# abdelhakim96/Dynamic-Obstacle-Avoidance-MPC

Measured on AMD Instinct MI355X. Metric: MPC solves/sec (N=20, 3 obstacles), higher is better.
Workload: dtype f64; 1 GPU; C2: 1024 identical scenarios per GPU, N=20, Tf=2s, 3 moving obstacles; global_batch=1024, per_gpu_batch=1024, N=20, n_obst=3, parallelism=single GPU

## Files before the change

### dynamic-obstacle-avoidance-mpc_amd/csrc/rti_split_kernel.hpp

```cpp
#pragma once
#include "rti_kernel.hpp"
#include <type_traits>

namespace mpc {

template <int LPS, int NOBST, bool W2 = false, bool BLK2 = false>
struct SplitLds {
    using LT = typename std::conditional<W2, RowLdsC, RowLds>::type;
    static constexpr int NBL = 6 / LPS;
    static constexpr int NSL = (NOBST + LPS - 1) / LPS;
    static __host__ __device__ constexpr int results(int N) { return W2 ? 0 : (N + 1) * RowLds::HS; }
    static __host__ __device__ constexpr int total(int N, bool lookahead)
    {
        if (BLK2) return Blk2Lds::total(N) + (lookahead ? (N + 1) * NOBST * 2 : 0);
        return LT::total(N, 1) + results(N) + ((lookahead && !W2) ? (N + 1) * NOBST * 2 : 0);
    }
};

template <int K>
__device__ __forceinline__ double nth_of_six(double a0, double a1, double a2, double a3, double a4, double a5)
{
    if constexpr (K == 0) return a0; else if constexpr (K == 1) return a1; else if constexpr (K == 2) return a2;
    else if constexpr (K == 3) return a3; else if constexpr (K == 4) return a4; else return a5;
}

#ifdef MPC_FORCE_WAVES2
#define MPC_SPLIT_BOUNDS(W2) __launch_bounds__(64, 2)
#else
#define MPC_SPLIT_BOUNDS(W2) __launch_bounds__(64, (W2) ? 2 : 1)
#endif
template <int NOBST, int LPS, bool W2 = false, bool MASKED = false, bool BLK2 = false, bool REF = false, bool IPAR = false, bool OSEL = false, bool IBND = false, bool NSQP = false>
__global__ MPC_SPLIT_BOUNDS(W2) void rti_split_kernel(const KParams p)
{
    static_assert(!NSQP || (IBND && !W2 && !BLK2), "the SQP loop is built on the per-instance bounds' code (dense blocks, one wavefront per SIMD)");
    static_assert(!IBND || OSEL, "the per-instance bounds are built on the obstacle masks' code");
    static_assert(!OSEL || (IPAR && MASKED), "the obstacle masks are built on the per-instance parameters' code with a run-time row count");
    static_assert(!REF || !BLK2, "the per-stage reference is not built for the block-2 recursions");
    static_assert(!IPAR || REF, "the per-instance parameters are built on the per-stage reference's code");
    static_assert(LPS == 2 || LPS == 3, "two or three lanes per horizon stage");
    static_assert(!BLK2 || !W2, "the block-2 recursions exist on the dense layout only");
    using SL = SplitLds<LPS, NOBST, W2, BLK2>;
    using LT = typename SL::LT;
    constexpr int NBL = SL::NBL, NSL = SL::NSL;
    constexpr int kKK = 45;
    const int lane = threadIdx.x;
    const int inst = p.order ? p.order[blockIdx.x] : (int)blockIdx.x;
    const int N = p.N;
    const int nact = MASKED ? p.n_obst : NOBST;
    const int i = lane / LPS;
    const int h = lane - i * LPS;
    const bool own = (h == 0);
    uint32_t omask = 0u;
    if constexpr (OSEL) omask = omask_word(p.omask, __builtin_amdgcn_readfirstlane(inst), nact);
    const int osub = OSEL ? 31 - __builtin_clz(omask | 1u) : 0;
#define OBST_ON(j) (OSEL ? (((omask >> (j)) & 1u) != 0u) : ((j) < nact))
#define OBST_IN(j) (OSEL ? ((((omask >> (j)) & 1u) != 0u) ? (j) : osub) : ((j) < nact ? (j) : nact - 1))
    const bool act = (i <= N);
    const bool has_u = (i < N);
    const bool xb = (i >= 1) && (i < N || (i == N && p.bx_terminal));
    const double dt = p.dt, h2 = p.h2;
    int is_part1 = (h == 1), is_part2 = (h == 2);
    asm volatile("" : "+v"(is_part1), "+v"(is_part2));
    auto part_of = [&](auto sc, double a0, double a1, double a2, double a3, double a4, double a5) {
        constexpr int s = decltype(sc)::value;
        double r = nth_of_six<s>(a0, a1, a2, a3, a4, a5);
        r = is_part1 ? nth_of_six<NBL + s>(a0, a1, a2, a3, a4, a5) : r;
        if (LPS == 3) r = is_part2 ? nth_of_six<(2 * NBL + s) % 6>(a0, a1, a2, a3, a4, a5) : r;
        return r;
    };
    auto zpart_of = [&](auto sc, double v0, double v1, double v2, double v3, double v5, double v6) {
        return part_of(sc, v0, v1, v2, v3, v5, v6);
    };
    using slot0 = std::integral_constant<int, 0>; using slot1 = std::integral_constant<int, 1>; using slot2 = std::integral_constant<int, 2>;
    auto slots_of = [&](const double (&v)[7], double (&out)[NBL]) {
        out[0] = zpart_of(slot0{}, v[0], v[1], v[2], v[3], v[5], v[6]);
        out[1] = zpart_of(slot1{}, v[0], v[1], v[2], v[3], v[5], v[6]);
        if constexpr (NBL > 2) out[2] = zpart_of(slot2{}, v[0], v[1], v[2], v[3], v[5], v[6]);
    };

#ifdef MPC_PHASE_TIMING
    long long tacc_[16] = {0, 0, 0, 0, 0, 0, 0, 0, 0, 0, 0, 0, 0, 0, 0, 0};
#endif
    MPC_T0();
    double x0v[5], gl[2];
#pragma unroll
    for (int c = 0; c < 5; c++) x0v[c] = p.x0[(size_t)inst * 5 + c];
    gl[0] = p.goal[(size_t)inst * 2]; gl[1] = p.goal[(size_t)inst * 2 + 1];
    if constexpr (W2) {
#pragma unroll
        for (int c = 0; c < 5; c++) x0v[c] = wave_uniform(x0v[c]);
        gl[0] = wave_uniform(gl[0]); gl[1] = wave_uniform(gl[1]);
    }
    double *Xg = p.X + (size_t)inst * (N + 1) * 5, *Ug = p.U + (size_t)inst * N * 2;
    const int ep_word = ((p.fused & kFuseMetrics) && p.ep_flags) ? p.ep_flags[inst] : 0;
    double xi[5] = {0, 0, 0, 0, 0}, ui[2] = {0, 0}, xnext[5] = {0, 0, 0, 0, 0};
    if (act) {
#pragma unroll
        for (int c = 0; c < 5; c++) xi[c] = Xg[i * 5 + c];
    }
    if (has_u) {
        ui[0] = Ug[i * 2]; ui[1] = Ug[i * 2 + 1];
#pragma unroll
        for (int c = 0; c < 5; c++) xnext[c] = Xg[(i + 1) * 5 + c];
    }
    extern __shared__ double lds_raw[];
    const LT RL = [&]() {
        if constexpr (W2) return RowLdsC(lds_raw + RowLdsC::CT + RowLdsC::pad_front(N), N, lds_raw);
        else return RowLds(lds_raw + RowLds::pad_front(N), N, lds_raw + RowLds::total(N, 1));
    }();
    const Blk2Lds BL(lds_raw, N);
    const RowLds RV(lds_raw, N / 2, BL.R);
    const int Mb = N >> 1;
    const int mblk = i >> 1;
    const bool odd = (i & 1) != 0;
    double *lds_P = BLK2 ? lds_raw + Blk2Lds::total(N) : (W2 ? RL.H : lds_raw + LT::total(N, 1) + SL::results(N));
    auto of_part = [&](double v, int q) { return q == 0 ? v : (q == 1 ? from_right(v) : from_right(from_right(v))); };
    constexpr bool FX = !W2 && !BLK2 && !(LPS == 2 && NOBST > 5);
    const bool obst_step = p.obst && (p.fused & (kFusePlant | kFuseObstacles | kFuseMetrics)) && lane < nact;
    double og[4] = {0, 0, 0, 0}, onz[2] = {0, 0};
    if constexpr (FX) {
        if (obst_step) {
            const double *o = p.obst + ((size_t)inst * nact + lane) * 4;
#pragma unroll
            for (int c = 0; c < 4; c++) og[c] = o[c];
            if ((p.fused & kFuseObstacles) && p.noise) { onz[0] = p.noise[((size_t)inst * nact + lane) * 2]; onz[1] = p.noise[((size_t)inst * nact + lane) * 2 + 1]; }
        }
    }
    double pxy[NSL][2];
    if (p.obst) {
        if (lane < 2 * nact) {
            const int j = lane >> 1, c = lane & 1;
            const double *o = p.obst + ((size_t)inst * nact + j) * 4;
            double q = o[c], v = (c == 0 && !p.world.bug_compat_predict) ? o[2] : o[3];
            const double lo = c ? p.world.ymin : p.world.xmin, hi = c ? p.world.ymax : p.world.xmax;
            lds_P[lane] = q;
            int k = 1;
            if constexpr (FX) {
                for (; k + 3 <= N; k += 4) {
                    double q4[4];
                    if (coord_advance4_clear(lo, hi, dt, q, v, q4)) q = q4[3];
                    else {
#pragma unroll
                        for (int j = 0; j < 4; j++) { coord_advance(lo, hi, dt, q, v); q4[j] = q; }
                    }
#pragma unroll
                    for (int j = 0; j < 4; j++) lds_P[(k + j) * NOBST * 2 + lane] = q4[j];
                }
            }
            for (; k <= N; k++) {
                coord_advance(lo, hi, dt, q, v);
                lds_P[k * NOBST * 2 + lane] = q;
            }
        }
        wave_sync();
    }
    MPC_TICK(10);
    if (p.obst) {
#pragma unroll
        for (int s = 0; s < NSL; s++) {
            const int j = s * LPS + h, jj = OBST_IN(j);
            const double *src = lds_P + ((act ? i : 0) * NOBST + jj) * 2;
            pxy[s][0] = src[0]; pxy[s][1] = src[1];
        }
    } else {
#pragma unroll
        for (int s = 0; s < NSL; s++) {
            const int j = s * LPS + h, jj = OBST_IN(j);
            const double *src = p.P + (((size_t)inst * (N + 1) + (act ? i : 0)) * nact + jj) * 2;
            pxy[s][0] = src[0]; pxy[s][1] = src[1];
        }
    }
    if constexpr (OSEL) {
        if (omask == 0u) {
#pragma unroll
            for (int s = 0; s < NSL; s++) { pxy[s][0] = 0.0; pxy[s][1] = 0.0; }
        }
    }
    if constexpr (FX) {
        if (p.obst) wave_sync();
        if (obst_step) {
            if (p.fused & kFuseObstacles) {
                if (p.noise) obstacle_noise(p.randomness, p.vmax, onz[0], onz[1], og[2], og[3]);
                obstacle_advance(p.world, dt, og[0], og[2], og[1], og[3]);
            }
            double *w = lds_P + 4 * lane;
#pragma unroll
            for (int c = 0; c < 4; c++) w[c] = og[c];
        }
    }
    const bool ep_done = (ep_word & 1) != 0;
    [[maybe_unused]] int sqp_k = 0, sqp_it = 0;
sqp_again: ;
    double fin = gl[0] + gl[1] + ui[0] + ui[1];
#pragma unroll
    for (int c = 0; c < 5; c++) fin += x0v[c] + xi[c] + xnext[c];
#pragma unroll
    for (int s = 0; s < NSL; s++) fin += pxy[s][0] + pxy[s][1];

    MPC_TICK(11);
    double zpen = 0.0;
    {
        const double ex = x0v[0] - gl[0], ey = x0v[1] - gl[1];
        const double scale = p.slack_a * (ex * ex + ey * ey + x0v[3] * x0v[3] + x0v[4] * x0v[4] + p.slack_b);
        const double alpha_i = p.alpha ? p.alpha[(size_t)inst * (N + 1) + (act ? i : N)] : scale * (double)(N - i) / (double)N;
        zpen = alpha_i * (has_u ? p.ss : 1.0);
    }
    const bool vs = act && (i >= 1) && (p.soft_h ? (zpen > 0.0) : true);
    const bool soft = p.soft_h != 0;

    double lin0 = 0.0;
    double d0[5] = {0, 0, 0, 0, 0};
    StageLin S;
    S.a02 = S.a03 = S.a04 = S.a12 = S.a13 = S.a14 = S.b00 = S.b01 = S.b10 = S.b11 = 0.0; S.dt = dt; S.h2 = h2;
    double bb[5] = {0, 0, 0, 0, 0};
    if (has_u) {
        double xn[5], ae[6], be[4];
        dyn_step<true>(xi, ui, dt, xn, ae, be);
        S.a02 = ae[0]; S.a03 = ae[1]; S.a04 = ae[2]; S.a12 = ae[3]; S.a13 = ae[4]; S.a14 = ae[5];
        S.b00 = be[0]; S.b01 = be[1]; S.b10 = be[2]; S.b11 = be[3];
#pragma unroll
        for (int c = 0; c < 5; c++) { bb[c] = xn[c] - xnext[c]; lin0 = fmax(lin0, fabs(bb[c])); }
    }
    if (i == 0) {
#pragma unroll
        for (int c = 0; c < 5; c++) { d0[c] = x0v[c] - xi[c]; lin0 = fmax(lin0, fabs(d0[c])); }
    }
    StageLin Sa = S;
    double bba[5] = {0, 0, 0, 0, 0}, bh0[5] = {0, 0, 0, 0, 0};
    if constexpr (BLK2) {
        if (own && has_u) {
            double *w = BL.S + 16 * i;
            w[0] = bb[2]; w[1] = bb[3]; w[2] = S.a02; w[3] = S.a03; w[4] = S.a04; w[5] = bb[0]; w[6] = S.b00; w[7] = S.b01;
            w[8] = bb[4]; w[9] = 0.0; w[10] = S.a12; w[11] = S.a13; w[12] = S.a14; w[13] = bb[1]; w[14] = S.b10; w[15] = S.b11;
        }
        wave_sync();
        if (act && odd) {
            const double *w = BL.S + 16 * (i - 1);
            Sa.a02 = w[2]; Sa.a03 = w[3]; Sa.a04 = w[4]; Sa.b00 = w[6]; Sa.b01 = w[7];
            Sa.a12 = w[10]; Sa.a13 = w[11]; Sa.a14 = w[12]; Sa.b10 = w[14]; Sa.b11 = w[15];
            bba[0] = w[5]; bba[1] = w[13]; bba[2] = w[0]; bba[3] = w[1]; bba[4] = w[8];
        }
        if (own && odd && has_u) {
            const double Wh[5][10] = {
                {1.0, 0.0, Sa.a02 + S.a02, Sa.a03 + S.a03, fma(S.a02, dt, Sa.a04) + S.a04, 0.0,
                 fma(S.a03, dt, Sa.b00), fma(S.a04, dt, fma(S.a02, h2, Sa.b01)), S.b00, S.b01},
                {0.0, 1.0, Sa.a12 + S.a12, Sa.a13 + S.a13, fma(S.a12, dt, Sa.a14) + S.a14, 0.0,
                 fma(S.a13, dt, Sa.b10), fma(S.a14, dt, fma(S.a12, h2, Sa.b11)), S.b10, S.b11},
                {0.0, 0.0, 1.0, 0.0, 2.0 * dt, 0.0, 0.0, fma(dt, dt, h2), 0.0, h2},
                {0.0, 0.0, 0.0, 1.0, 0.0, 0.0, dt, 0.0, dt, 0.0},
                {0.0, 0.0, 0.0, 0.0, 1.0, 0.0, 0.0, dt, 0.0, dt}};
            double *w = BL.W + Blk2Lds::WS * mblk;
#pragma unroll
            for (int k = 0; k < 5; k++)
#pragma unroll
                for (int c = 0; c < 10; c++) w[k * 10 + c] = Wh[k][c];
            bh0[0] = fma(S.a04, bba[4], fma(S.a03, bba[3], fma(S.a02, bba[2], bba[0]))) + bb[0];
            bh0[1] = fma(S.a14, bba[4], fma(S.a13, bba[3], fma(S.a12, bba[2], bba[1]))) + bb[1];
            bh0[2] = fma(dt, bba[4], bba[2]) + bb[2]; bh0[3] = bba[3] + bb[3]; bh0[4] = bba[4] + bb[4];
        }
        if (own && act && (odd || i == N)) {
            double *hc = BL.H + Blk2Lds::HS * mblk;
#pragma unroll
            for (int e = 0; e < 100; e++) hc[e] = 0.0;
        }
    } else
    if constexpr (W2) {
        if (own && act) { double *hc = RL.H + LT::HS * i; hc[49] = 0.0; hc[50] = 0.0; }
        if (lane < 8) {
            const double c2[8] = {0.0, 0.0, 1.0, 0.0, dt, 0.0, 0.0, h2}, c3[8] = {0.0, 0.0, 0.0, 1.0, 0.0, 0.0, dt, 0.0}, c4[8] = {0.0, 0.0, 0.0, 0.0, 1.0, 0.0, 0.0, dt};
            double v2 = 0.0, v3 = 0.0, v4 = 0.0;
// ... 31 lines not shown
    double cl0[NBL], ch0[NBL], hq[NBL], hd[NBL], gc0[NBL];
    double ll[NBL], tl[NBL], lh[NBL], th[NBL], rtl[NBL], rth[NBL], zs[NBL];
    double yr[REF ? 6 : 1];
    if constexpr (IPAR) load_ref_or_goal<IPAR>(p.yref, p.ref_off, p.ref_T, inst, act ? i : N, has_u, gl, yr);
    else if constexpr (REF) load_ref(p, inst, act ? i : N, has_u, yr);
    IpConst *const ipw = IPAR ? ip_const(p.ip_w, (size_t)__builtin_amdgcn_readfirstlane(inst) * kIpW) : nullptr;
#define ROW_R2(s) (IPAR ? p.ip_r2[(size_t)inst * nact + (OSEL ? OBST_IN((s) * LPS + h) : ((s) * LPS + h < nact ? (s) * LPS + h : nact - 1))] : p.r2)
    IpConst *const ipb = IBND ? ip_const(p.ip_b, (size_t)__builtin_amdgcn_readfirstlane(inst) * kIpB) : nullptr;
    {
        auto slot_init = [&](auto sc) {
            constexpr int s = decltype(sc)::value;
            const double val = part_of(sc, ui[0], ui[1], xi[0], xi[1], xi[3], xi[4]);
            double lo, hi;
            if constexpr (IBND) {
                lo = part_of(sc, ipb[kIpBuLo + 0], ipb[kIpBuLo + 1], ipb[kIpBxLo + 0], ipb[kIpBxLo + 1], ipb[kIpBxLo + 2], ipb[kIpBxLo + 3]);
                hi = part_of(sc, ipb[kIpBuHi + 0], ipb[kIpBuHi + 1], ipb[kIpBxHi + 0], ipb[kIpBxHi + 1], ipb[kIpBxHi + 2], ipb[kIpBxHi + 3]);
            } else {
                lo = part_of(sc, p.bu_lo[0], p.bu_lo[1], p.bx_lo[0], p.bx_lo[1], p.bx_lo[2], p.bx_lo[3]);
                hi = part_of(sc, p.bu_hi[0], p.bu_hi[1], p.bx_hi[0], p.bx_hi[1], p.bx_hi[2], p.bx_hi[3]);
            }
            const bool is_u = part_of(sc, 1.0, 1.0, 0.0, 0.0, 0.0, 0.0) != 0.0;
            bp[s] = act && (is_u ? has_u : xb);
            if constexpr (IPAR)
                hd[s] = part_of(sc, has_u ? ipw[kIpHs + 0] : 0.0, has_u ? ipw[kIpHs + 1] : 0.0, has_u ? ipw[kIpHs + 2] : ipw[kIpHt + 0],
                                has_u ? ipw[kIpHs + 3] : ipw[kIpHt + 1], has_u ? ipw[kIpHs + 5] : ipw[kIpHt + 3], has_u ? ipw[kIpHs + 6] : ipw[kIpHt + 4]);
            else
                hd[s] = part_of(sc, has_u ? p.Hd_stage[0] : 0.0, has_u ? p.Hd_stage[1] : 0.0, has_u ? p.Hd_stage[2] : p.Hd_term[0],
                                has_u ? p.Hd_stage[3] : p.Hd_term[1], has_u ? p.Hd_stage[5] : p.Hd_term[3], has_u ? p.Hd_stage[6] : p.Hd_term[4]);
            hq[s] = (is_u && !has_u) ? 1.0 : hd[s];
            double wg;
            if constexpr (IPAR)
                wg = part_of(sc, has_u ? ipw[kIpWg + 4] : 0.0, has_u ? ipw[kIpWg + 5] : 0.0, has_u ? ipw[kIpWg + 0] : ipw[kIpWe + 0], has_u ? ipw[kIpWg + 1] : ipw[kIpWe + 1],
                             has_u ? ipw[kIpWg + 2] : ipw[kIpWe + 2], has_u ? ipw[kIpWg + 3] : ipw[kIpWe + 3]);
            else
                wg = part_of(sc, has_u ? p.Wg[4] : 0.0, has_u ? p.Wg[5] : 0.0, has_u ? p.Wg[0] : p.Weg[0], has_u ? p.Wg[1] : p.Weg[1],
                             has_u ? p.Wg[2] : p.Weg[2], has_u ? p.Wg[3] : p.Weg[3]);
            if constexpr (REF) gc0[s] = wg * (val - part_of(sc, yr[4], yr[5], yr[0], yr[1], yr[2], yr[3]));
            else gc0[s] = wg * (val - part_of(sc, 0.0, 0.0, gl[0], gl[1], 0.0, 0.0));
            cl0[s] = val - lo; ch0[s] = hi - val;
            tl[s] = fmax(cl0[s], p.thr0); th[s] = fmax(ch0[s], p.thr0);
            rtl[s] = rcp_nr(tl[s]); rth[s] = rcp_nr(th[s]);
            ll[s] = p.mu0 * rtl[s]; lh[s] = p.mu0 * rth[s];
            zs[s] = 0.0;
            if (bp[s]) lin0 = fmax(lin0, fmax(tl[s] - cl0[s], th[s] - ch0[s]));
        };
        slot_init(std::integral_constant<int, 0>{});
        slot_init(std::integral_constant<int, 1>{});
        if constexpr (NBL > 2) slot_init(std::integral_constant<int, 2>{});
    }
    double hd_psi_;
    if constexpr (IPAR) hd_psi_ = has_u ? ipw[kIpHs + 4] : ipw[kIpHt + 2];
    else hd_psi_ = has_u ? p.Hd_stage[4] : p.Hd_term[2];
    const double hd_psi = hd_psi_;
    bool sp[NSL];
    double hh[NSL], ax[NSL], ay[NSL], sv[NSL], l1[NSL], t1[NSL], l2[NSL], t2[NSL], rt1[NSL], rt2[NSL];
#pragma unroll
    for (int s = 0; s < NSL; s++) {
        if constexpr (OSEL) sp[s] = vs && OBST_ON(s * LPS + h);
        else sp[s] = vs && (s * LPS + h < nact);
        const double ex = xi[0] - pxy[s][0], ey = xi[1] - pxy[s][1];
        hh[s] = ex * ex + ey * ey - ROW_R2(s); ax[s] = 2 * ex; ay[s] = 2 * ey;
        if (soft) {
            sv[s] = (hh[s] < 0 ? -hh[s] : 0.0) + p.thr0;
            t1[s] = fmax(hh[s] + sv[s], p.thr0);
            t2[s] = fmax(sv[s], p.thr0);
        } else {
            sv[s] = 0.0; t1[s] = fmax(hh[s], p.thr0); t2[s] = 1.0;
            if (sp[s]) lin0 = fmax(lin0, t1[s] - hh[s]);
        }
        rt1[s] = rcp_nr(t1[s]); rt2[s] = rcp_nr(t2[s]);
        l1[s] = p.mu0 * rt1[s]; l2[s] = soft ? p.mu0 * rt2[s] : 0.0;
    }
    int n_items_lane = 0;
#pragma unroll
    for (int s = 0; s < NBL; s++) n_items_lane += bp[s] ? 2 : 0;
#pragma unroll
    for (int s = 0; s < NSL; s++) n_items_lane += sp[s] ? (soft ? 2 : 1) : 0;
    const double n_items = seg_sum<64>((double)n_items_lane, lane);
    const double inv_items = wave_uniform(n_items > 0 ? 1.0 / n_items : 0.0);
    if (!(fabs(fin) <= 1e300)) lin0 = INFINITY;
    lin0 = wave_uniform(seg_max<64>(lin0, lane));

    double z[7] = {0, 0, 0, 0, 0, 0, 0};
    double rhoPi = 1.0;
    int it = 0;
    IpmState ipm;
    ipm.running = !ep_done;
    int &status = ipm.status, &it_done = ipm.it_done;
    bool &running = ipm.running;
    float stepl = 0.0f;
    if (!(lin0 <= 1e300)) { status = 4; running = false; }

    auto stationarity = [&]() {
        double gsh[NBL], gk[6] = {0, 0, 0, 0, 0, 0}, sx = 0.0, sy = 0.0, rsm = 0.0;
#pragma unroll
        for (int s = 0; s < NBL; s++) { gsh[s] = gc0[s] + hd[s] * zs[s] + (bp[s] ? lh[s] - ll[s] : 0.0); gk[s] = gsh[s]; }
#pragma unroll
        for (int s = 0; s < NSL; s++) if (sp[s]) {
            sx -= l1[s] * ax[s]; sy -= l1[s] * ay[s];
            if (soft) rsm = fmax(rsm, fabs(zpen * sv[s] + zpen - l1[s] - l2[s]));
        }
        double shx = sx, shy = sy;
#pragma unroll
        for (int q = 1; q < LPS; q++) {
#pragma unroll
            for (int s = 0; s < NBL; s++) gsh[s] = from_right(gsh[s]);
// ... 39 lines not shown
        double rdl[NBL], rdh[NBL];
        struct SoftT { double w1, w2, rD, be1, be2, rs, rd1, rd2; } so[NSL];
        double hdiag_[NBL], g_[NBL], ssum[5];
        {
#pragma unroll
            for (int s = 0; s < NBL; s++) {
                rdl[s] = (cl0[s] + zs[s]) - tl[s];
                rdh[s] = (ch0[s] - zs[s]) - th[s];
                double hdiag = hq[s], g = gc0[s] + hd[s] * zs[s];
                if (bp[s]) {
                    const double wl = ll[s] * rtl[s], wh = lh[s] * rth[s];
                    const double bl = (ll[s] * tl[s] + ll[s] * rdl[s]) * rtl[s], bh = (lh[s] * th[s] + lh[s] * rdh[s]) * rth[s];
                    hdiag += wl + wh;
                    g += lh[s] - ll[s];
                    g += bl - bh;
                }
                hdiag_[s] = hdiag; g_[s] = g;
            }
            double sxx = 0.0, syy = 0.0, sxy = 0.0, glx = 0.0, gly = 0.0, cbx = 0.0, cby = 0.0;
#pragma unroll
            for (int s = 0; s < NSL; s++) {
                SoftT &o = so[s];
                const double y = ax[s] * z[2] + ay[s] * z[3];
                o.w1 = l1[s] * rt1[s];
                if (soft) {
                    o.rd1 = (hh[s] + y + sv[s]) - t1[s]; o.rd2 = sv[s] - t2[s];
                    o.be1 = (l1[s] * t1[s] + l1[s] * o.rd1) * rt1[s];
                    o.w2 = l2[s] * rt2[s];
                    o.be2 = (l2[s] * t2[s] + l2[s] * o.rd2) * rt2[s];
                    o.rs = zpen * sv[s] + zpen - l1[s] - l2[s];
                    o.rD = rcp_nr(zpen + o.w1 + o.w2);
                } else {
                    o.rd1 = (hh[s] + y) - t1[s]; o.rd2 = 0.0;
                    o.be1 = (l1[s] * t1[s] + l1[s] * o.rd1) * rt1[s];
                    o.w2 = 0.0; o.be2 = 0.0; o.rs = 0.0; o.rD = 0.0;
                }
                if (sp[s]) {
                    double weff, geff;
                    if (soft) {
                        weff = o.w1 * (zpen + o.w2) * o.rD;
                        geff = (o.be1 * (zpen + o.w2) - o.w1 * (o.rs + o.be2)) * o.rD;
                    } else { weff = o.w1; geff = o.be1; }
                    sxx += weff * ax[s] * ax[s]; syy += weff * ay[s] * ay[s]; sxy += weff * ax[s] * ay[s];
                    glx -= l1[s] * ax[s]; gly -= l1[s] * ay[s];
                    cbx += geff * ax[s]; cby += geff * ay[s];
                }
            }
            ssum[0] = sxx; ssum[1] = syy; ssum[2] = sxy; ssum[3] = glx + cbx; ssum[4] = gly + cby;
        }
        MPC_TICK(1);
        double bbr[5], x_init[5];
#pragma unroll
        for (int c = 0; c < 5; c++) { bbr[c] = rhoPi * bb[c]; x_init[c] = rhoPi * d0[c]; }
        {
            double Hk[6], gk[6], Ssum[5], sh_h[NBL], sh_g[NBL], sh_s[5];
#pragma unroll
            for (int s = 0; s < NBL; s++) { Hk[s] = hdiag_[s]; gk[s] = g_[s]; sh_h[s] = hdiag_[s]; sh_g[s] = g_[s]; }
#pragma unroll
            for (int e = 0; e < 5; e++) { Ssum[e] = ssum[e]; sh_s[e] = ssum[e]; }
#pragma unroll
            for (int q = 1; q < LPS; q++) {
#pragma unroll
                for (int s = 0; s < NBL; s++) { sh_h[s] = from_right(sh_h[s]); sh_g[s] = from_right(sh_g[s]); }
#pragma unroll
                for (int e = 0; e < 5; e++) sh_s[e] = from_right(sh_s[e]);
#pragma unroll
                for (int s = 0; s < NBL; s++) { Hk[q * NBL + s] = sh_h[s]; gk[q * NBL + s] = sh_g[s]; }
#pragma unroll
                for (int e = 0; e < 5; e++) Ssum[e] += sh_s[e];
            }
            const double Sxx = Ssum[0], Syy = Ssum[1], Sxy = Ssum[2], Sgx = Ssum[3], Sgy = Ssum[4];
            if constexpr (BLK2) {
                const double q[5] = {Hk[2] + Sxx, Hk[3] + Syy, hd_psi, Hk[4], Hk[5]};
                const double g[5] = {gk[2] + Sgx, gk[3] + Sgy, hd_psi * z[4], gk[4], gk[5]};
                const double r0 = Hk[0], r1 = Hk[1], lu0 = gk[0], lu1 = gk[1];
                if (own && act && !odd && i < N) {
                    double *x = BL.R + Blk2Lds::RS * mblk;
#pragma unroll
                    for (int c = 0; c < 5; c++) { x[c] = q[c]; x[5 + c] = g[c]; }
                    x[10] = Sxy; x[11] = r0; x[12] = r1; x[13] = lu0; x[14] = lu1;
                }
                if (own && i == N) {
                    double *hc = BL.H + Blk2Lds::HS * mblk;
#pragma unroll
                    for (int c = 0; c < 5; c++) { hc[11 * c] = q[c]; hc[10 * c + 5] = g[c]; hc[50 + c] = g[c]; }
                    hc[1] = Sxy; hc[10] = Sxy;
                }
                wave_sync();
                if (own && odd && act) {
                    const double *x = BL.R + Blk2Lds::RS * mblk;
                    double qa[5], ga[5];
#pragma unroll
                    for (int c = 0; c < 5; c++) { qa[c] = x[c]; ga[c] = x[5 + c]; }
                    const double qaxy = x[10], ra0 = x[11], ra1 = x[12], lua0 = x[13], lua1 = x[14];
                    const double C0[7] = {1.0, 0.0, Sa.a02, Sa.a03, Sa.a04, Sa.b00, Sa.b01}, C1[7] = {0.0, 1.0, Sa.a12, Sa.a13, Sa.a14, Sa.b10, Sa.b11};
                    double s0[7], s1[7];
                    s0[0] = q[0]; s0[1] = Sxy; s1[0] = Sxy; s1[1] = q[1];
#pragma unroll
                    for (int c = 2; c < 7; c++) { s0[c] = fma(q[0], C0[c], Sxy * C1[c]); s1[c] = fma(Sxy, C0[c], q[1] * C1[c]); }
                    double Y[7][7];
#pragma unroll
                    for (int c = 0; c < 7; c++) { Y[0][c] = s0[c]; Y[1][c] = s1[c]; }
#pragma unroll
                    for (int r = 2; r < 7; r++)
#pragma unroll
                        for (int c = r; c < 7; c++) Y[r][c] = fma(C0[r], s0[c], C1[r] * s1[c]);
// ... 113 lines not shown
        if constexpr (BLK2) {
            rowpar_factor2(lane, Mb, BL, lane < 16);
            wave_sync();
            if (has_u) {
                const double *ko = BL.R + Blk2Lds::RS * mblk;
#pragma unroll
                for (int u = 0; u < 4; u++) {
#pragma unroll
                    for (int c = 0; c < 5; c++) Kh[u][c] = ko[8 * u + c];
                    kh[u] = ko[8 * u + 5];
                }
                if (own && odd) {
#pragma unroll
                    for (int e = 0; e < 10; e++) fac[e] = ko[Blk2Lds::FAC + e];
                }
            }
            if (own && odd && has_u) {
                const double B0[4] = {fma(S.a03, dt, Sa.b00), fma(S.a04, dt, fma(S.a02, h2, Sa.b01)), S.b00, S.b01};
                const double B1[4] = {fma(S.a13, dt, Sa.b10), fma(S.a14, dt, fma(S.a12, h2, Sa.b11)), S.b10, S.b11};
                const double A0[5] = {1.0, 0.0, Sa.a02 + S.a02, Sa.a03 + S.a03, fma(S.a02, dt, Sa.a04) + S.a04};
                const double A1[5] = {0.0, 1.0, Sa.a12 + S.a12, Sa.a13 + S.a13, fma(S.a12, dt, Sa.a14) + S.a14};
                const double h2d = fma(dt, dt, h2);
                double *acl = BL.R + Blk2Lds::RS * mblk + RowVec::ACL;
#pragma unroll
                for (int c = 0; c < 6; c++) {
                    const double k0 = c < 5 ? Kh[0][c] : kh[0], k1 = c < 5 ? Kh[1][c] : kh[1], k2 = c < 5 ? Kh[2][c] : kh[2], k3 = c < 5 ? Kh[3][c] : kh[3];
                    const double a0 = c < 5 ? A0[c] : rhoPi * bh0[0], a1 = c < 5 ? A1[c] : rhoPi * bh0[1];
                    const double a2 = c < 5 ? (c == 2 ? 1.0 : (c == 4 ? 2.0 * dt : 0.0)) : rhoPi * bh0[2];
                    const double a3 = c < 5 ? (c == 3 ? 1.0 : 0.0) : rhoPi * bh0[3], a4 = c < 5 ? (c == 4 ? 1.0 : 0.0) : rhoPi * bh0[4];
                    acl[0 * RowVec::RS + c] = fma(B0[3], k3, fma(B0[2], k2, fma(B0[1], k1, fma(B0[0], k0, a0))));
                    acl[1 * RowVec::RS + c] = fma(B1[3], k3, fma(B1[2], k2, fma(B1[1], k1, fma(B1[0], k0, a1))));
                    acl[2 * RowVec::RS + c] = fma(h2, k3, fma(h2d, k1, a2));
                    acl[3 * RowVec::RS + c] = fma(dt, k2, fma(dt, k0, a3));
                    acl[4 * RowVec::RS + c] = fma(dt, k3, fma(dt, k1, a4));
                }
            }
            MPC_TICK(2);
            if (lane == 0) {
#pragma unroll
                for (int c = 0; c < 5; c++) BL.R[RowVec::X + c] = x_init[c];
            }
            wave_sync();
            MPC_TICK(3);
            rowpar_vector_fast<true>(lane, Mb, RV, lane < 16);
            MPC_TICK(15);
            wave_sync();
            pair_step(bbra, za);
            MPC_TICK(3);
        } else {
#ifdef MPC_MFMA4
        if constexpr (!W2) mfma4_factor(lane, N, RL); else
#endif
        {
            constexpr bool kSixRows = W2 || (NOBST == 10 && LPS == 2 && !MASKED && REF && IPAR && !OSEL);
            rowpar_factor<LT, (LT::COMPACT ? kSweepTermsCopied : kSweepTermsOutOfPlace), kSixRows>(lane, N, RL, lane < 16, dt);
        }
        wave_sync();
        if (has_u) {
            const double *ko = RL.R + LT::HS * i;
#pragma unroll
            for (int c = 0; c < 5; c++) { F.K0[c] = ko[c]; F.K1[c] = ko[8 + c]; }
            F.k0 = ko[5]; F.k1 = ko[13]; F.i00 = ko[6]; F.l = ko[7]; F.i11 = ko[14];
        }
        if (own && has_u) {
            double *acl = RL.R + LT::HS * i + RowVec::ACL;
            const double Ar[2][5] = {{1.0, 0.0, S.a02, S.a03, S.a04}, {0.0, 1.0, S.a12, S.a13, S.a14}};
            const double Br[2][2] = {{S.b00, S.b01}, {S.b10, S.b11}};
#pragma unroll
            for (int c = 0; c < 5; c++) {
                acl[0 * RowVec::RS + c] = Ar[0][c] + Br[0][0] * F.K0[c] + Br[0][1] * F.K1[c];
                acl[1 * RowVec::RS + c] = Ar[1][c] + Br[1][0] * F.K0[c] + Br[1][1] * F.K1[c];
                acl[2 * RowVec::RS + c] = (c == 2 ? 1.0 : (c == 4 ? dt : 0.0)) + h2 * F.K1[c];
                acl[3 * RowVec::RS + c] = (c == 3 ? 1.0 : 0.0) + dt * F.K0[c];
                acl[4 * RowVec::RS + c] = (c == 4 ? 1.0 : 0.0) + dt * F.K1[c];
            }
            double *cc = acl + 5;
            cc[0 * RowVec::RS] = bbr[0] + S.b00 * F.k0 + S.b01 * F.k1; cc[1 * RowVec::RS] = bbr[1] + S.b10 * F.k0 + S.b11 * F.k1;
            cc[2 * RowVec::RS] = bbr[2] + h2 * F.k1; cc[3 * RowVec::RS] = bbr[3] + dt * F.k0; cc[4 * RowVec::RS] = bbr[4] + dt * F.k1;
        }
        MPC_TICK(2);
        if (lane == 0) {
#pragma unroll
            for (int c = 0; c < 5; c++) RL.R[RowVec::X + c] = x_init[c];
        }
        wave_sync();
        MPC_TICK(3);
        rowpar_vector_fast<true>(lane, N, RL, lane < 16);
        MPC_TICK(15);
        wave_sync();
        if (act) {
            const double *xx = RL.R + LT::HS * i + RowVec::X;
            double u0 = F.k0, u1 = F.k1;
#pragma unroll
            for (int c = 0; c < 5; c++) { za[2 + c] = xx[c]; u0 += F.K0[c] * xx[c]; u1 += F.K1[c] * xx[c]; }
            za[0] = u0; za[1] = u1;
        }
        MPC_TICK(3);

        }

        double ppl[NBL], pph[NBL], pp1[NSL], pp2[NSL];
        double smu;
        {
            double rmax = 0.0, rmaxd = 0.0;
            double dtl_[NBL], dth_[NBL], dll_[NBL], dlh_[NBL], zas[NBL];
            slots_of(za, zas);
#pragma unroll
            for (int s = 0; s < NBL; s++) {
                const double dzk = zas[s];
                dtl_[s] = dzk + rdl[s]; dth_[s] = -dzk + rdh[s];
                dll_[s] = -(ll[s] * tl[s] + ll[s] * dtl_[s]) * rtl[s]; dlh_[s] = -(lh[s] * th[s] + lh[s] * dth_[s]) * rth[s];
                ppl[s] = dll_[s] * dtl_[s]; pph[s] = dlh_[s] * dth_[s];
                if (bp[s]) {
                    rmax = fmax(rmax, fmax(-dtl_[s] * rtl[s], -dth_[s] * rth[s]));
                    rmaxd = fmax(rmaxd, fmax(fma(dtl_[s], rtl[s], 1.0), fma(dth_[s], rth[s], 1.0)));
                }
// ... 256 lines not shown
        const double *xg = p.x0 + (size_t)inst * 5, *gg = p.goal + (size_t)inst * 2;
        asm volatile("" : "+v"(xg), "+v"(gg));
#pragma unroll
        for (int c = 0; c < 5; c++) x0v[c] = xg[c];
        gl[0] = gg[0]; gl[1] = gg[1];
    }
    if constexpr (NSQP) {
        status = ipm_finite_step<64>(status, z, lane);
        tail_full_step(status, z, xi, ui);
        sqp_k += 1; sqp_it += it_done;
        const double nrm = wave_uniform(seg_max<64>(sqp_step_norm(act, has_u, z), lane));
        if (!ep_done && status != 4 && sqp_k < p.sqp_max && !(nrm <= p.sqp_tol)) {
#pragma unroll
            for (int c = 0; c < 5; c++) {
                xi[c] = act ? xi[c] : 0.0;
                double r = from_right(xi[c]);
#pragma unroll
                for (int q = 1; q < LPS; q++) r = from_right(r);
                xnext[c] = has_u ? r : 0.0;
            }
            ui[0] = has_u ? ui[0] : 0.0; ui[1] = has_u ? ui[1] : 0.0;
            goto sqp_again;
        }
        it_done = sqp_it;
    }
    if constexpr (FX) {
        const bool store = !ep_done;
        const bool lane0s = (lane == 0) && store;
        double ox = 0.0, oy = 0.0, ovx = 0.0, ovy = 0.0;
        if (obst_step) {
            const double *w = lds_P + 4 * lane;
            ox = w[0]; oy = w[1]; ovx = w[2]; ovy = w[3];
        }
        int acc_it = 0, acc_st = 0, ep_fl = 0, ep_inc = 0;
        double ep_mm = 0.0;
        if (lane0s) {
            if (p.iters_acc) acc_it = p.iters_acc[inst];
            if (p.status_acc) acc_st = p.status_acc[inst];
            if (p.fused & kFuseMetrics) { ep_fl = p.ep_flags[inst]; ep_mm = p.ep_min_margin[inst]; }
        }
        if constexpr (!NSQP) {
        status = ipm_finite_step<64>(status, z, lane);
        tail_full_step(status, z, xi, ui);
        }
        const double u_apply[2] = {lane_value(ui[0], 0), lane_value(ui[1], 0)};
        tail_reset_on_fail(p.fused, status, x0v, gl[1], i, N, xi, ui);
        const bool fused_step = (p.fused & (kFusePlant | kFuseObstacles | kFuseMetrics)) != 0;
        double xnew[5] = {x0v[0], x0v[1], x0v[2], x0v[3], x0v[4]};
        if (fused_step) {
            double xp[5] = {x0v[0], x0v[1], x0v[2], x0v[3], x0v[4]};
            if ((p.fused & kFuseAliasBug) && (p.fused & kFuseResetOnFail) && status == 4) { xp[3] = 0.0; xp[4] = 0.0; }
#pragma unroll
            for (int c = 0; c < 5; c++) xnew[c] = xp[c];
            if (p.fused & kFusePlant) dyn_step<false>(xp, u_apply, dt, xnew, nullptr, nullptr);
            double margin = INFINITY;
            if (obst_step) {
                const double ddx = xnew[0] - ox, ddy = xnew[1] - oy;
                margin = sqrt(ddx * ddx + ddy * ddy) - (IPAR ? p.ip_rhit[(size_t)inst * nact + lane] : p.r_hit);
                if constexpr (OSEL) {
                    if (!OBST_ON(lane) && !(p.fused & kFuseMarginAll)) margin = INFINITY;
                }
            }
            if (p.fused & kFuseMetrics) {
                margin = -seg_max<64>(-margin, lane);
                if (lane0s) {
                    if (xnew[0] < p.world.xmin || xnew[0] > p.world.xmax || xnew[1] < p.world.ymin || xnew[1] > p.world.ymax) ep_fl |= 2;
                    ep_mm = fmin(ep_mm, margin);
                    if (ep_mm <= 0.0) ep_fl |= 4;
                    const double gx_ = xnew[0] - gl[0], gy_ = xnew[1] - gl[1];
                    if (sqrt(gx_ * gx_ + gy_ * gy_) <= p.tol_goal) ep_fl |= 1;
                    else ep_inc = 1;
                }
            }
        }
        double J = 0.0;
        if (p.cost) {
            if (act) {
                if (IPAR && own) {
                    double r[6];
                    load_ref_or_goal<IPAR>(p.yref, p.ref_off, p.ref_T, inst, i, has_u, gl, r);
                    const double wg[6] = {ipw[kIpWg], ipw[kIpWg + 1], ipw[kIpWg + 2], ipw[kIpWg + 3], ipw[kIpWg + 4], ipw[kIpWg + 5]};
                    const double we[4] = {ipw[kIpWe], ipw[kIpWe + 1], ipw[kIpWe + 2], ipw[kIpWe + 3]};
                    J = ls_cost_ref(wg, we, xi, ui, r, has_u);
                } else if (REF && own) {
                    const double *row = ref_row(p.yref, p.ref_off, p.ref_T, inst, i);
                    const double r[6] = {row[0], row[1], row[2], row[3], has_u ? row[4] : 0.0, has_u ? row[5] : 0.0};
                    J = ls_cost_ref(p.Wg, p.Weg, xi, ui, r, has_u);
                } else if (own) {
                    const double ex = xi[0] - gl[0], ey = xi[1] - gl[1];
                    if (has_u) J = 0.5 * (p.Wg[0] * ex * ex + p.Wg[1] * ey * ey + p.Wg[2] * xi[3] * xi[3] + p.Wg[3] * xi[4] * xi[4]
                                          + p.Wg[4] * ui[0] * ui[0] + p.Wg[5] * ui[1] * ui[1]);
                    else J = 0.5 * (p.Weg[0] * ex * ex + p.Weg[1] * ey * ey + p.Weg[2] * xi[3] * xi[3] + p.Weg[3] * xi[4] * xi[4]);
                }
#pragma unroll
                for (int s = 0; s < NSL; s++) if (OBST_ON(s * LPS + h)) {
                    const double dx = xi[0] - pxy[s][0], dy = xi[1] - pxy[s][1];
                    const double hv = dx * dx + dy * dy - ROW_R2(s);
                    const double v = hv < 0 ? -hv : 0.0;
                    J += zpen * (v + 0.5 * v * v);
                }
            }
            J = seg_sum<64>(J, lane);
        }
        if (store && own && (status != 4 || (p.fused & (kFuseResetOnFail | kFuseShift)))) tail_store_iterate(p.fused, i, N, act, has_u, xi, ui, Xg, Ug);
        if (fused_step) {
            if ((p.fused & kFusePlant) && lane0s && p.x0_rw) {
#pragma unroll
// ... 126 lines not shown
```

Baseline: 7.667 million solves/s.

## Spread dynamics quadrature, Hessian staging and closed-loop rows across lanes of each stage

Each lane of a horizon stage now computes only its share of the Gauss-Legendre quadrature sincos nodes and exchanges them with neighbours through cross-lane moves. This replaces every lane evaluating all four nodes redundantly in the linearisation and the plant step. Hessian and gradient staging into LDS and the closed-loop A+BK rows are also split so each lane writes its own entries, where one owner lane used to build everything. This trims redundant transcendental and serial work per stage, at the cost of extra cross-lane shuffles, selects and more intricate index bookkeeping that could be wrong for some template configurations.

```diff
diff --git a/dynamic-obstacle-avoidance-mpc_amd/csrc/rti_split_kernel.hpp b/dynamic-obstacle-avoidance-mpc_amd/csrc/rti_split_kernel.hpp
--- a/dynamic-obstacle-avoidance-mpc_amd/csrc/rti_split_kernel.hpp
+++ b/dynamic-obstacle-avoidance-mpc_amd/csrc/rti_split_kernel.hpp
@@ -22,6 +22,91 @@
 {
     if constexpr (K == 0) return a0; else if constexpr (K == 1) return a1; else if constexpr (K == 2) return a2;
     else if constexpr (K == 3) return a3; else if constexpr (K == 4) return a4; else return a5;
+}
+
+__device__ __forceinline__ void dyn_step_quad(const double x[5], const double u[2], double dt, int lane, double xn[5])
+{
+    const double psi = x[2], v = x[3], om = x[4], a = u[0], al = u[1];
+    double vj[4], pj[4], w[4];
+#pragma unroll
+    for (int j = 0; j < 4; j++) {
+        const double tau = kGLC[j] * dt;
+        w[j] = kGLB[j] * dt;
+        vj[j] = v + a * tau;
+        pj[j] = psi + om * tau + 0.5 * al * tau * tau;
+    }
+    const int k = lane & 3;
+    double arg = pj[0];
+    arg = (k == 1) ? pj[1] : arg; arg = (k == 2) ? pj[2] : arg; arg = (k == 3) ? pj[3] : arg;
+    double sk, ck;
+    sincos(arg, &sk, &ck);
+    const double sn[4] = {dpp_f64<0x00>(sk), dpp_f64<0x55>(sk), dpp_f64<0xAA>(sk), dpp_f64<0xFF>(sk)};
+    const double cn[4] = {dpp_f64<0x00>(ck), dpp_f64<0x55>(ck), dpp_f64<0xAA>(ck), dpp_f64<0xFF>(ck)};
+    double sx = 0, sy = 0;
+#pragma unroll
+    for (int j = 0; j < 4; j++) {
+        const double wvc = w[j] * vj[j] * cn[j], wvs = w[j] * vj[j] * sn[j];
+        sx += wvc; sy += wvs;
+    }
+    xn[0] = x[0] + sx; xn[1] = x[1] + sy;
+    xn[2] = psi + om * dt + 0.5 * al * dt * dt;
+    xn[3] = v + a * dt;
+    xn[4] = om + al * dt;
+}
+template <int LPS>
+__device__ __forceinline__ void dyn_step_parts(const double x[5], const double u[2], double dt, int is_part1, int is_part2, double xn[5], double ae[6], double be[4])
+{
+    const double psi = x[2], v = x[3], om = x[4], a = u[0], al = u[1];
+    double pj[4];
+#pragma unroll
+    for (int j = 0; j < 4; j++) {
+        const double tau = kGLC[j] * dt;
+        pj[j] = psi + om * tau + 0.5 * al * tau * tau;
+    }
+    double sn[4], cn[4];
+    if constexpr (LPS == 3) {
+        double arg = pj[0];
+        arg = is_part1 ? pj[1] : arg; arg = is_part2 ? pj[2] : arg;
+        double sh, ch;
+        sincos(arg, &sh, &ch);
+        sincos(pj[3], &sn[3], &cn[3]);
+        const double sr = from_right(sh), cr = from_right(ch), sl = from_left(sh), cl = from_left(ch);
+        const double srr = from_right(sr), crr = from_right(cr), sll = from_left(sl), cll = from_left(cl);
+        sn[0] = is_part2 ? sll : (is_part1 ? sl : sh); cn[0] = is_part2 ? cll : (is_part1 ? cl : ch);
+        sn[1] = is_part2 ? sl : (is_part1 ? sh : sr);  cn[1] = is_part2 ? cl : (is_part1 ? ch : cr);
+        sn[2] = is_part2 ? sh : (is_part1 ? sr : srr); cn[2] = is_part2 ? ch : (is_part1 ? cr : crr);
+    } else {
+        double sa, ca, sb, cb;
+        sincos(is_part1 ? pj[1] : pj[0], &sa, &ca);
+        sincos(is_part1 ? pj[3] : pj[2], &sb, &cb);
+        const double sal = from_left(sa), cal = from_left(ca), sar = from_right(sa), car = from_right(ca);
+        const double sbl = from_left(sb), cbl = from_left(cb), sbr = from_right(sb), cbr = from_right(cb);
+        sn[0] = is_part1 ? sal : sa; cn[0] = is_part1 ? cal : ca;
+        sn[1] = is_part1 ? sa : sar; cn[1] = is_part1 ? ca : car;
+        sn[2] = is_part1 ? sbl : sb; cn[2] = is_part1 ? cbl : cb;
+        sn[3] = is_part1 ? sb : sbr; cn[3] = is_part1 ? cb : cbr;
+    }
+    double sx = 0, sy = 0, xpsi = 0, xv = 0, xom = 0, xa = 0, xal = 0, ypsi = 0, yv = 0, yom = 0, ya = 0, yal = 0;
+#pragma unroll
+    for (int j = 0; j < 4; j++) {
+        const double tau = kGLC[j] * dt, w = kGLB[j] * dt;
+        const double vj = v + a * tau;
+        const double sj = sn[j], cj = cn[j];
+        const double wvc = w * vj * cj, wvs = w * vj * sj;
+        sx += wvc; sy += wvs;
+        const double ht2 = 0.5 * tau * tau;
+        xpsi -= wvs;        ypsi += wvc;
+        xv += w * cj;       yv += w * sj;
+        xom -= wvs * tau;   yom += wvc * tau;
+        xa += w * tau * cj; ya += w * tau * sj;
+        xal -= wvs * ht2;   yal += wvc * ht2;
+    }
+    xn[0] = x[0] + sx; xn[1] = x[1] + sy;
+    xn[2] = psi + om * dt + 0.5 * al * dt * dt;
+    xn[3] = v + a * dt;
+    xn[4] = om + al * dt;
+    ae[0] = xpsi; ae[1] = xv; ae[2] = xom; ae[3] = ypsi; ae[4] = yv; ae[5] = yom;
+    be[0] = xa; be[1] = xal; be[2] = ya; be[3] = yal;
 }
 
 #ifdef MPC_FORCE_WAVES2
@@ -116,6 +201,16 @@
     double *lds_P = BLK2 ? lds_raw + Blk2Lds::total(N) : (W2 ? RL.H : lds_raw + LT::total(N, 1) + SL::results(N));
     auto of_part = [&](double v, int q) { return q == 0 ? v : (q == 1 ? from_right(v) : from_right(from_right(v))); };
     constexpr bool FX = !W2 && !BLK2 && !(LPS == 2 && NOBST > 5);
+    constexpr bool kNodesDealt = !W2 && !NSQP && !(NOBST == 10 && LPS == 2 && !MASKED && REF && IPAR && !OSEL);
+    constexpr bool kSixRows = W2 || (NOBST == 10 && LPS == 2 && !MASKED && REF && IPAR && !OSEL);
+#ifdef MPC_MFMA4
+    constexpr bool kRow5Staged = true;
+#else
+    constexpr bool kRow5Staged = kSixRows;
+#endif
+    constexpr bool kStagingDealt = !W2 && !BLK2 && !NSQP;
+    constexpr bool kAclDealt = LPS == 3 && !W2 && !BLK2 && !NSQP;
+    constexpr bool kPlantDealt = FX && !NSQP;
     const bool obst_step = p.obst && (p.fused & (kFusePlant | kFuseObstacles | kFuseMetrics)) && lane < nact;
     double og[4] = {0, 0, 0, 0}, onz[2] = {0, 0};
     if constexpr (FX) {
@@ -215,7 +310,8 @@
     double bb[5] = {0, 0, 0, 0, 0};
     if (has_u) {
         double xn[5], ae[6], be[4];
-        dyn_step<true>(xi, ui, dt, xn, ae, be);
+        if constexpr (kNodesDealt) dyn_step_parts<LPS>(xi, ui, dt, is_part1, is_part2, xn, ae, be);
+        else dyn_step<true>(xi, ui, dt, xn, ae, be);
         S.a02 = ae[0]; S.a03 = ae[1]; S.a04 = ae[2]; S.a12 = ae[3]; S.a13 = ae[4]; S.a14 = ae[5];
         S.b00 = be[0]; S.b01 = be[1]; S.b10 = be[2]; S.b11 = be[3];
 #pragma unroll
@@ -353,6 +449,9 @@
     if constexpr (IPAR) hd_psi_ = has_u ? ipw[kIpHs + 4] : ipw[kIpHt + 2];
     else hd_psi_ = has_u ? p.Hd_stage[4] : p.Hd_term[2];
     const double hd_psi = hd_psi_;
+    if constexpr (kStagingDealt) {
+        if (own && act) RL.H[LT::HS * i + 18] = hd_psi;
+    }
     bool sp[NSL];
     double hh[NSL], ax[NSL], ay[NSL], sv[NSL], l1[NSL], t1[NSL], l2[NSL], t2[NSL], rt1[NSL], rt2[NSL];
 #pragma unroll
@@ -498,6 +597,50 @@
         double bbr[5], x_init[5];
 #pragma unroll
         for (int c = 0; c < 5; c++) { bbr[c] = rhoPi * bb[c]; x_init[c] = rhoPi * d0[c]; }
+        if constexpr (kStagingDealt) {
+            double *hc = RL.H + LT::HS * i;
+            const double gpsi = hd_psi * z[4];
+            if constexpr (LPS == 3) {
+                double Sm[5];
+#pragma unroll
+                for (int e = 0; e < 5; e++) { const double l = from_left(ssum[e]), r = from_right(ssum[e]); Sm[e] = (l + ssum[e]) + r; }
+                if (act) {
+                    if (h == 1) {
+                        const double gx = g_[0] + Sm[3], gy = g_[1] + Sm[4];
+                        hc[0] = hdiag_[0] + Sm[0]; hc[1] = Sm[2]; hc[8] = Sm[2]; hc[9] = hdiag_[1] + Sm[1]; hc[5] = gx; hc[13] = gy;
+                        if constexpr (kRow5Staged) { hc[40] = gx; hc[41] = gy; }
+                    } else if (h == 2) {
+                        hc[27] = hdiag_[0]; hc[36] = hdiag_[1]; hc[21] = gpsi; hc[29] = g_[0]; hc[37] = g_[1];
+                        if constexpr (kRow5Staged) { hc[42] = gpsi; hc[43] = g_[0]; hc[44] = g_[1]; }
+                    } else {
+                        hc[54] = hdiag_[0]; hc[63] = hdiag_[1]; hc[53] = g_[0]; hc[61] = g_[1];
+                        if constexpr (kRow5Staged) { hc[46] = g_[0]; hc[47] = g_[1]; }
+                        if (has_u) {
+#pragma unroll
+                            for (int k = 0; k < 5; k++) RL.W[LT::WS * i + k * 8 + 5] = bbr[k];
+                        }
+                    }
+                }
+            } else {
+                const double Sxx = ssum[0] + from_right(ssum[0]), Sxy = ssum[2] + from_right(ssum[2]), Sgx = ssum[3] + from_right(ssum[3]);
+                const double Syy = from_left(ssum[1]) + ssum[1], Sgy = from_left(ssum[4]) + ssum[4];
+                if (act) {
+                    if (h == 1) {
+                        const double gy = g_[0] + Sgy;
+                        hc[9] = hdiag_[0] + Syy; hc[27] = hdiag_[1]; hc[36] = hdiag_[2]; hc[13] = gy; hc[21] = gpsi; hc[29] = g_[1]; hc[37] = g_[2];
+                        if constexpr (kRow5Staged) { hc[41] = gy; hc[42] = gpsi; hc[43] = g_[1]; hc[44] = g_[2]; }
+                        if (has_u) {
+#pragma unroll
+                            for (int k = 0; k < 5; k++) RL.W[LT::WS * i + k * 8 + 5] = bbr[k];
+                        }
+                    } else {
+                        const double gx = g_[2] + Sgx;
+                        hc[54] = hdiag_[0]; hc[63] = hdiag_[1]; hc[0] = hdiag_[2] + Sxx; hc[1] = Sxy; hc[8] = Sxy; hc[53] = g_[0]; hc[61] = g_[1]; hc[5] = gx;
+                        if constexpr (kRow5Staged) { hc[46] = g_[0]; hc[47] = g_[1]; hc[40] = gx; }
+                    }
+                }
+            }
+        } else
         {
             double Hk[6], gk[6], Ssum[5], sh_h[NBL], sh_g[NBL], sh_s[5];
 #pragma unroll
@@ -717,7 +860,6 @@
         if constexpr (!W2) mfma4_factor(lane, N, RL); else
 #endif
         {
-            constexpr bool kSixRows = W2 || (NOBST == 10 && LPS == 2 && !MASKED && REF && IPAR && !OSEL);
             rowpar_factor<LT, (LT::COMPACT ? kSweepTermsCopied : kSweepTermsOutOfPlace), kSixRows>(lane, N, RL, lane < 16, dt);
         }
         wave_sync();
@@ -727,6 +869,21 @@
             for (int c = 0; c < 5; c++) { F.K0[c] = ko[c]; F.K1[c] = ko[8 + c]; }
             F.k0 = ko[5]; F.k1 = ko[13]; F.i00 = ko[6]; F.l = ko[7]; F.i11 = ko[14];
         }
+        if constexpr (kAclDealt) {
+            if (has_u) {
+                const double *ko = RL.R + LT::HS * i + h;
+                const double Ka0 = ko[0], Kb0 = ko[3], Ka1 = ko[8], Kb1 = ko[11];
+                const double Aa[5] = {is_part2 ? S.a02 : (is_part1 ? 0.0 : 1.0), is_part2 ? S.a12 : (is_part1 ? 1.0 : 0.0), is_part2 ? 1.0 : 0.0, 0.0, 0.0};
+                const double Ab[5] = {is_part2 ? bbr[0] : (is_part1 ? S.a04 : S.a03), is_part2 ? bbr[1] : (is_part1 ? S.a14 : S.a13),
+                                      is_part2 ? bbr[2] : (is_part1 ? dt : 0.0), is_part2 ? bbr[3] : (is_part1 ? 0.0 : 1.0), is_part2 ? bbr[4] : (is_part1 ? 1.0 : 0.0)};
+                double *acl = RL.R + LT::HS * i + RowVec::ACL + h;
+                acl[0 * RowVec::RS] = Aa[0] + S.b00 * Ka0 + S.b01 * Ka1; acl[0 * RowVec::RS + 3] = Ab[0] + S.b00 * Kb0 + S.b01 * Kb1;
+                acl[1 * RowVec::RS] = Aa[1] + S.b10 * Ka0 + S.b11 * Ka1; acl[1 * RowVec::RS + 3] = Ab[1] + S.b10 * Kb0 + S.b11 * Kb1;
+                acl[2 * RowVec::RS] = Aa[2] + h2 * Ka1;                  acl[2 * RowVec::RS + 3] = Ab[2] + h2 * Kb1;
+                acl[3 * RowVec::RS] = Aa[3] + dt * Ka0;                  acl[3 * RowVec::RS + 3] = Ab[3] + dt * Kb0;
+                acl[4 * RowVec::RS] = Aa[4] + dt * Ka1;                  acl[4 * RowVec::RS + 3] = Ab[4] + dt * Kb1;
+            }
+        } else
         if (own && has_u) {
             double *acl = RL.R + LT::HS * i + RowVec::ACL;
             const double Ar[2][5] = {{1.0, 0.0, S.a02, S.a03, S.a04}, {0.0, 1.0, S.a12, S.a13, S.a14}};
@@ -1089,7 +1246,10 @@
             if ((p.fused & kFuseAliasBug) && (p.fused & kFuseResetOnFail) && status == 4) { xp[3] = 0.0; xp[4] = 0.0; }
 #pragma unroll
             for (int c = 0; c < 5; c++) xnew[c] = xp[c];
-            if (p.fused & kFusePlant) dyn_step<false>(xp, u_apply, dt, xnew, nullptr, nullptr);
+            if (p.fused & kFusePlant) {
+                if constexpr (kPlantDealt) dyn_step_quad(xp, u_apply, dt, lane, xnew);
+                else dyn_step<false>(xp, u_apply, dt, xnew, nullptr, nullptr);
+            }
             double margin = INFINITY;
             if (obst_step) {
                 const double ddx = xnew[0] - ox, ddy = xnew[1] - oy;
```

Measured after the change: 7.905 million solves/s (median of 6 runs). +3.1%, better.
